# Robotics-Engineer-khy/ti5_isaacgym

Hardware: AMD Instinct MI355X
Metric: env-steps/sec at 8192 envs, t1_dh_stand, 1/2/4/8 MI355X; obs/reward parity (higher is better)
Workload: dtype f32

## Files before the change

ti5_isaacgym_amd/csrc/t1env_dyn6.hip:

```cpp
#include <hip/hip_runtime.h>

#define T1_CONTACT_ONE_COPY

#ifdef T1_PROBE_SIMD
__device__ unsigned g_t1_simd6[4096][8];
#endif
#ifdef T1_PROBE_CLOCK
__device__ unsigned long long g_t1_clock6[4];
constexpr int T1_WGSUM6_N = 4 + 6;
__device__ unsigned long long g_t1_wgtime6[4096][4];
__device__ unsigned long long g_t1_wgsum6[4096][T1_WGSUM6_N];
#define T1_CLOCK_WAIT_BEGIN() const unsigned long long t1c_w0 = __builtin_amdgcn_s_memtime();
#define T1_CLOCK_SHIFT_END(wi)                                                     \
  if ((threadIdx.x & 63) == 0 && blockIdx.x < 4096 && (wi) >= 0)                   \
    atomicAdd(&g_t1_wgsum6[blockIdx.x][4 + (wi)], __builtin_amdgcn_s_memtime() - t1c_w0);
#define T1_CLOCK_LOOP_END()                                                        \
  if (threadIdx.x == 0 && blockIdx.x < 4096) g_t1_wgtime6[blockIdx.x][3] = __builtin_amdgcn_s_memrealtime();
#define T1_CLOCK_WAIT_END(k)                                                       \
  if (threadIdx.x == 0 && blockIdx.x < 4096)                                       \
    atomicAdd(&g_t1_wgsum6[blockIdx.x][k], __builtin_amdgcn_s_memtime() - t1c_w0);
#define T1_CLOCK_BEGIN()                                                           \
  unsigned long long t1c_cyc0 = 0, t1c_rt0 = 0;                                    \
  if (threadIdx.x == 0) {                                                          \
    t1c_cyc0 = __builtin_amdgcn_s_memtime();                                       \
    t1c_rt0 = __builtin_amdgcn_s_memrealtime();                                    \
    if (blockIdx.x < 4096) { g_t1_wgtime6[blockIdx.x][0] = t1c_rt0; g_t1_wgtime6[blockIdx.x][2] = 0; } \
  }
#define T1_CLOCK_END()                                                             \
  if (threadIdx.x == 0) {                                                          \
    const unsigned long long c1 = __builtin_amdgcn_s_memtime(), r1 = __builtin_amdgcn_s_memrealtime(); \
    atomicAdd(&g_t1_clock6[0], c1 - t1c_cyc0);                                     \
    atomicAdd(&g_t1_clock6[1], r1 - t1c_rt0);                                      \
    atomicAdd(&g_t1_clock6[2], 1ull);                                              \
    if (blockIdx.x < 4096) {                                                       \
      g_t1_wgtime6[blockIdx.x][1] = r1;                                            \
      atomicAdd(&g_t1_wgsum6[blockIdx.x][0], c1 - t1c_cyc0);                       \
    }                                                                              \
  }                                                                                \
  T1_CLOCK_WAVE_END();
#define T1_CLOCK_WAVE_END()                                                        \
  if ((threadIdx.x & 63) == 0 && blockIdx.x < 4096)                                \
    atomicMax(&g_t1_wgtime6[blockIdx.x][2], (unsigned long long)__builtin_amdgcn_s_memrealtime());
constexpr int T1_TAIL6_N = 16;
__device__ unsigned long long g_t1_tail6[4096][T1_TAIL6_N];
#define T1_CLOCK_STAMP(k)                                                          \
  if ((threadIdx.x & 63) == 0 && blockIdx.x < 4096)                                \
    g_t1_tail6[blockIdx.x][k] = __builtin_amdgcn_s_memrealtime();
#else
#define T1_CLOCK_BEGIN() ((void)0)
#define T1_CLOCK_END() ((void)0)
#define T1_CLOCK_WAVE_END() ((void)0)
#define T1_CLOCK_WAIT_BEGIN() ((void)0)
#define T1_CLOCK_WAIT_END(k) ((void)0)
#define T1_CLOCK_SHIFT_END(wi) ((void)0)
#define T1_CLOCK_LOOP_END() ((void)0)
#define T1_CLOCK_STAMP(k) ((void)0)
#endif

#define T1_PROF_WAVES 8
#define T1_PROF_NAME(x) x##6
#include "t1env_prof.h"

#include "t1_dyn5.h"
#include "t1env_device.h"
#include "t1env_internal.h"
#include "t1env_postphys.h"
// ... 14 lines not shown
constexpr int SHIFT6_WAVES = __builtin_popcount(SHIFT6_MASK);
static_assert((SHIFT6_MASK & 0x11) == 0, "W0 / W4 (the core chain's SIMD) do not shift");

struct Dyn6Lds {
  DynModel model;
  Rows4<Q_N> st;
  Rows4<WB_N> wb;
  SubspaceRows sj;
  Rows4<R_N> w1;
  Rows4<XCH> wc[WC_N];
  PdStage<64> pd;
  float cap[CAP5_N][64];
  float act[12][NE6];
  float epi[EPI_N][NE6];
  float fr[FR_N][NE6];
  float vish[64];
  float vift[64];
  float amx[4][64];
  LegParams<float> pl[64];
  BaseParams<float> pb[64];
  float rtf[2][3][64];
  float rsf[2][3][64];
  uint32_t e2;
};
T1_ROWS_ALIGNED(Dyn6Lds, st);
T1_ROWS_ALIGNED(Dyn6Lds, wb);
T1_ROWS_ALIGNED(Dyn6Lds, sj);
T1_ROWS_ALIGNED(Dyn6Lds, w1);
T1_ROWS_ALIGNED(Dyn6Lds, wc);
static_assert(sizeof(Rows4<XCH>) % 16 == 0 && alignof(Dyn6Lds) % 16 == 0, "every wc[i], and the struct itself");

template <int F, int H, bool HALF>
__device__ __forceinline__ void shift_chunk_elems(const uint8_t* in0, uint8_t* out0, uint32_t i, uint32_t nel) {
  constexpr uint32_t ROW = F * H, PER = HALF ? 8 : 4;
#pragma unroll 1
  for (uint32_t k = 0; k < PER; ++k) {
    const uint32_t e = i + k;
    if (e < nel && e % ROW < ROW - F) {
      if constexpr (HALF)
        reinterpret_cast<uint16_t*>(out0)[e] = reinterpret_cast<const uint16_t*>(in0)[e + F];
      else
        reinterpret_cast<float*>(out0)[e] = reinterpret_cast<const float*>(in0)[e + F];
    }
  }
}
template <int F, int H, bool HALF>
__device__ __forceinline__ void shp_range(int64_t total, int64_t r0, int64_t r1, int sl, int nsl, uint32_t& lo,
// ... 492 lines not shown
    halves(vi_b, vl, vr);
    __syncthreads();
    V3<float> fb = v3<float>(0.0f, 0.0f, 0.0f);
    {
      BaseState<float> sb;
      float q[NLEG], qd[NLEG];
      read_state_rows(lds.st, lane, sb, q, qd);
      if (leg == 0) {
      BaseFrame<float> F;
      base_frame(sb, F);
      const float vt0 = restitution_target(M, eg, vl), vt1 = restitution_target(M, eg, vr);
      fb = body_contact_force(M, T, 0, F.R0, v3<float>(0, 0, 0), F.abs, F.V0, mu, vt0 > vt1 ? vt0 : vt1);
      }
    }
    __syncthreads();
    if (leg == 0) {
      if (active) {
        float* cf = B.contact_forces + (size_t)n * 39;
        cf[0] = fb.x; cf[1] = fb.y; cf[2] = fb.z;
      }
      if constexpr (FUSED) { lds.fr[F_CFB][e] = fb.x; lds.fr[F_CFB + 1][e] = fb.y; lds.fr[F_CFB + 2][e] = fb.z; }
    }
    T1_PROF_MARK(10);
    if constexpr (FUSED) __syncthreads();
    T1_CLOCK_WAVE_END();
    T1_PROF_END();
    return;
  }

  if (role != 0) {
    T1_PROF_MARK(21);
    const int wi = shift6_index(role);
    const float mu = 0.5f * (B.friction[n] + M.ground_friction);
    const float mu_self = B.friction[n];
    const float eg = ground_restitution(M, B.restitution[n]);
    if (FUSED && wave >= 4) stage_epilogue_inputs<NE6, 256>(B, N, (int)r0, (int)threadIdx.x - 256, lds.epi);
    T1_PROF_MARK(22);
    const int bsh = 1 + 6 * leg + K_SHANK, bft = 1 + 6 * leg + K_FOOT;
    const int half = role >= 4 ? 1 : 0;
    if (role == 1) {
      LegParams<float> PL;
      load_leg_params(M, B, n, j0, PL);
      ShiftHold hold;
      ShiftWalk walk;
      shp_begin(S, r0, r1, nsub, wi, lane, walk, hold);
      for (int sub = 0; sub < nsub; ++sub) {
        T1_PROF_MARK(4);
// ... 164 lines not shown
            const float w[3] = {lds.cap[2 * NLEG + 4][lane], lds.cap[2 * NLEG + 5][lane], lds.cap[2 * NLEG + 6][lane]};
            capture_imu(quat, w, imu_dst);
          }
        }
      }
      __syncthreads();
      T1_PROF_MARK(11);
      if (role == 6) {
        float* cf = B.contact_forces + (size_t)n * 39;
#pragma unroll
        for (int s = 0; s < 2; ++s) {
          const int b = s == 0 ? bsh : bft;
          const float f[3] = {lds.rtf[s][0][lane] + lds.rsf[s][0][lane], lds.rtf[s][1][lane] + lds.rsf[s][1][lane],
                              lds.rtf[s][2][lane] + lds.rsf[s][2][lane]};
          if (active) { cf[b * 3 + 0] = f[0]; cf[b * 3 + 1] = f[1]; cf[b * 3 + 2] = f[2]; }
          if (FUSED && s == 1) {
            const int r = leg == 0 ? F_C0 : F_C1;
            lds.fr[r][e] = f[0]; lds.fr[r + 1][e] = f[1]; lds.fr[r + 2][e] = f[2];
          }
        }
      }
    }
    if constexpr (FUSED) {
      if (role == 1 && lane == 0) lds.e2 = 0u;
      __syncthreads();
      T1_PROF_MARK(12);
      if (role == 1)
        fused_epilogue_staged<POST_A_STATE, NE6, true, false>(M, C, B, A, S, FA, dyn_blocks, lane, lds.epi,
                                                                             lds.fr, lds.act, lds.act + NLEG, &lds.e2);
      else if (role == 2)
        fused_epilogue_obs<POST_OBS_PRIV, NE6>(M, C, B, A, lane, lds.epi, lds.fr, lds.act, lds.act + NLEG);
      else if (role == 3)
        fused_epilogue_obs<POST_OBS_ACTOR, NE6>(M, C, B, A, lane, lds.epi, lds.fr, lds.act, lds.act + NLEG);
      else if (wave >= 5)
        epilogue_zero_reset_rows<NE6>(C, B, S, lane, (int)threadIdx.x - 320, 192, lds.epi, lds.fr);
      T1_PROF_MARK(15);
    }
    T1_CLOCK_WAVE_END();
    T1_PROF_END();
    return;
  }

  BaseParams<float>& PB = lds.pb[lane];
  LegParams<float>& PL = lds.pl[lane];
  {
    BaseState<float> sb;
    float q[NLEG], qd[NLEG];
    BaseParams<float> pb;
    LegParams<float> pl;
    load_base_params(M, B, n, pb);
    load_leg_params(M, B, n, j0, pl);
    load_base_state(M, pb, B.root_states + (size_t)n * 13, sb);
    PB = pb;
    PL = pl;
#pragma unroll
    for (int k = 0; k < NLEG; ++k) {
      q[k] = B.dof_state[n * 24 + 2 * (j0 + k)];
      qd[k] = B.dof_state[n * 24 + 2 * (j0 + k) + 1];
// ... 120 lines not shown
  }
  float (*FR)[NE6] = FUSED ? lds.fr : nullptr;
  if constexpr (FUSED) {
#pragma unroll
    for (int k = 0; k < NLEG; ++k) {
      lds.fr[F_DOF + 2 * (j0 + k)][e] = q[k];
      lds.fr[F_DOF + 2 * (j0 + k) + 1][e] = qd[k];
    }
  }
  T1_PROF_MARK(8);
  __syncthreads();
  T1_PROF_MARK(9);
  {
    BaseFrame<float> F;
    base_frame(sb, F);
    leg_report_rigid<NE6>(M, B, PB, sb, F, q, qd, no, leg, active, e, FR);
  }
  T1_PROF_MARK(10);
  __syncthreads();
  T1_PROF_MARK(11);
  if constexpr (FUSED) {
    __syncthreads();
    T1_PROF_MARK(12);
    fused_epilogue_staged<POST_A_REWARDS, NE6, true, false>(M, C, B, A, S, FA, dyn_blocks, lane, lds.epi,
                                                                           lds.fr, lds.act, lds.act + NLEG, &lds.e2);
  }
  T1_CLOCK_END();
  T1_PROF_END();
}

#ifdef T1_PROBE_SIMD
extern "C" int t1env_debug_simd6(unsigned* out, int blocks) {
  return (int)hipMemcpyFromSymbol(out, HIP_SYMBOL(g_t1_simd6), sizeof(unsigned) * 8 * (size_t)blocks);
}
#endif

#ifdef T1_PROBE_CLOCK
extern "C" int t1env_debug_wgtime6(unsigned long long* out, int blocks) {
  return (int)hipMemcpyFromSymbol(out, HIP_SYMBOL(g_t1_wgtime6), sizeof(unsigned long long) * 4 * (size_t)blocks);
}
extern "C" int t1env_debug_tail6(unsigned long long* out, int blocks) {
  return (int)hipMemcpyFromSymbol(out, HIP_SYMBOL(g_t1_tail6), sizeof(unsigned long long) * T1_TAIL6_N * (size_t)blocks);
}
extern "C" int t1env_debug_wgsum6(unsigned long long* out, int blocks, int reset) {
  hipError_t e = hipMemcpyFromSymbol(out, HIP_SYMBOL(g_t1_wgsum6), sizeof(unsigned long long) * T1_WGSUM6_N * (size_t)blocks);
  if (e == hipSuccess && reset) {
    static unsigned long long zero[4096][T1_WGSUM6_N] = {};
    e = hipMemcpyToSymbol(HIP_SYMBOL(g_t1_wgsum6), zero, sizeof(zero));
// ... 29 lines not shown
```

ti5_isaacgym_amd/csrc/t1env_fused.h:

```cpp
#pragma once
#include "t1env_device.h"
#include "t1env_internal.h"
#include "t1env_postphys.h"

#ifndef T1_CLOCK_STAMP
#define T1_CLOCK_STAMP(k) ((void)0)
#endif

namespace t1 {

constexpr int SHIFT_UNIT = 8;
constexpr int K_SHANK = 3, K_FOOT = 5;
static_assert(T1_LEG_CONTACT_MASK == ((1 << K_SHANK) | (1 << K_FOOT)), "the step kernels assume shank + foot contacts");
constexpr int XCH = 27;

constexpr uint32_t HANDOFF_SHIFT = 1u, HANDOFF_DYN = 2u;
__device__ __forceinline__ uint32_t unit_handoff(uint32_t* word, uint32_t epoch, uint32_t bits) {
  const uint32_t tag = (epoch & 0x3fffffu) << 10;
  uint32_t old = __hip_atomic_load(word, __ATOMIC_RELAXED, __HIP_MEMORY_SCOPE_AGENT);
  for (;;) {
    const uint32_t nw = ((old & ~0x3ffu) == tag ? old : tag) | bits;
    if (__hip_atomic_compare_exchange_strong(word, &old, nw, __ATOMIC_RELAXED, __ATOMIC_RELAXED,
                                             __HIP_MEMORY_SCOPE_AGENT))
      return nw;
// ... 242 lines not shown
  while (todo) {
    const int l = __ffsll(todo) - 1;
    todo &= todo - 1;
    const int64_t row = (int64_t)blockIdx.x * NE + l;
    zero_history_row(S, row, t, nt);
    zero_span_wide(B.act_hist + row * 48, 48, t, nt);
    zero_span_wide(B.dof_hist + row * 96, 96, t, nt);
    zero_span_wide(B.imu_hist + row * 16, 16, t, nt);
  }
}

__device__ __forceinline__ void epilogue_reset_rest(const DynModel& M, const t1env_config& C, const t1env_buffers& B,
                                                    const t1env_step_args& A, int n, uint32_t genv, uint32_t ctr,
                                                    RngKey K, const float (&cmd)[4], float org[3], bool org_known,
                                                    bool zero_lag_rings) {
  reset_env_rest(M, C, B, n, K, org, org_known, false, true, zero_lag_rings);
  ObsIn O;
#pragma unroll
  for (int i = 0; i < 4; ++i) O.cmd[i] = cmd[i];
  reset_obs_inputs(M, C, K, O, false);
  if (resample_commands_r(C, A, O.el, O.gt, O.cmd, genv, ctr)) strow(B.commands + n * 4, O.cmd);
}

template <int PART, int NE, bool INWG, bool RESET_ROWS = true>
__device__ __forceinline__ void fused_epilogue_staged(const DynModel& M, const t1env_config& C, const t1env_buffers& B,
                                                      const t1env_step_args& A, const ShiftArgs& S,
                                                      const FusedArgs& FA, int dyn_blocks, int lane,
                                                      const float (*E)[NE], const float (*FR)[NE],
                                                      const float (*ACT0)[NE], const float (*ACT1)[NE],
                                                      uint32_t* e2_flag = nullptr) {
  const int N = C.num_envs;
  constexpr int TS = PART == POST_A_REWARDS ? 0 : 8;
  T1_CLOCK_STAMP(TS);
  const int e = lane % NE;
  const int n0 = lane < NE ? (int)blockIdx.x * NE + lane : N;
  const bool active = n0 < N;
  const int n = active ? n0 : N - 1;
  PostAIn X;
#pragma unroll
  for (int i = 0; i < 13; ++i) X.root[i] = FR[F_ROOT + i][e];
#pragma unroll
  for (int i = 0; i < 24; ++i) X.dof[i] = FR[F_DOF + i][e];
#pragma unroll
  for (int i = 0; i < 13; ++i) { X.f0[i] = FR[F_F0 + i][e]; X.f1[i] = FR[F_F1 + i][e]; }
#pragma unroll
  for (int i = 0; i < 2; ++i) { X.k0[i] = FR[F_K0 + i][e]; X.k1[i] = FR[F_K1 + i][e]; }
#pragma unroll
  for (int i = 0; i < 3; ++i) { X.cfb[i] = FR[F_CFB + i][e]; X.c0[i] = FR[F_C0 + i][e]; X.c1[i] = FR[F_C1 + i][e]; }
#pragma unroll
  for (int i = 0; i < 12; ++i) X.tq[i] = FR[F_TQ + i][e];
#pragma unroll
  for (int k = 0; k < NLEG; ++k) { X.a[k] = ACT0[k][e]; X.a[NLEG + k] = ACT1[k][e]; }
#pragma unroll
  for (int i = 0; i < 12; ++i) {
    X.la[i] = E[E_LA + i][e]; X.lla[i] = E[E_LLA + i][e];
    X.ldv[i] = E[E_LDV + i][e]; X.ref[i] = E[E_REF + i][e];
// ... 3 lines not shown
#pragma unroll
  for (int i = 0; i < 4; ++i) X.cmd[i] = E[E_CMD + i][e];
#pragma unroll
  for (int i = 0; i < 2; ++i) {
    X.at[i] = E[E_AT + i][e]; X.fh[i] = E[E_FH + i][e]; X.lfz[i] = E[E_LFZ + i][e];
    X.lc[i] = (uint8_t)__float_as_int(E[E_LC + i][e]);
  }
#pragma unroll
  for (int i = 0; i < 3; ++i) {
    X.ef[i] = E[E_EF + i][e]; X.et[i] = E[E_ET + i][e];
    X.gt[i] = __float_as_int(E[E_GT + i][e]);
  }
#pragma unroll
  for (int k = 0; k < T1_NREW; ++k) X.esum[k] = E[E_ESUM + k][e];
  X.el = (int64_t)(((uint64_t)(uint32_t)__float_as_int(E[E_EL + 1][e]) << 32) |
                   (uint32_t)__float_as_int(E[E_EL][e]));
  X.pl = (int64_t)(((uint64_t)(uint32_t)__float_as_int(E[E_PL + 1][e]) << 32) |
                   (uint32_t)__float_as_int(E[E_PL][e]));
  X.gstart = E[E_GS][e];
  BaseQ bq;
  float* const ep_row = FA.ep_part + (size_t)blockIdx.x * EP_PART_ROW;
  const bool in_level_sum = PART == POST_A_STATE && C.custom_origins && active;
  int level = in_level_sum ? B.terrain_levels[n] : 0;
  const bool do_reset = post_a_core<PART>(M, C, B, A, n0, X, bq, PART == POST_A_REWARDS ? ep_row : nullptr);
  T1_PROF_MARK(13);
  T1_CLOCK_STAMP(TS + 1);
  if constexpr (PART == POST_A_REWARDS) {
    if constexpr (RESET_ROWS) epilogue_handoff<NE, INWG>(C, S, FA, lane, do_reset, active);
    T1_CLOCK_STAMP(TS + 2);
    __builtin_amdgcn_s_waitcnt(0);
    T1_CLOCK_STAMP(TS + 3);
    if (e2_flag) {
      while (__hip_atomic_load(e2_flag, __ATOMIC_ACQUIRE, __HIP_MEMORY_SCOPE_WORKGROUP) == 0u) __builtin_amdgcn_s_sleep(1);
    } else {
      __syncthreads();
    }
    T1_CLOCK_STAMP(TS + 4);
    epilogue_finalize_parts(C, B, A, FA, dyn_blocks, lane);
    T1_CLOCK_STAMP(TS + 5);
    T1_PROF_MARK(15);
    return;
  }
  const uint32_t genv = (uint32_t)(C.env_offset + n);
  const uint32_t ctr = A.counter + 1u;
  const RngKey K = rng_key(C.seed, genv, ctr);
  float org[3];
  bool org_known = false;
  if (active && do_reset) {
    const float pos_cmd[4] = {X.root[0], X.root[1], X.cmd[0], X.cmd[1]};
    org_known = reset_curriculum(C, B, n, K, true, pos_cmd, org, level, in_level_sum);
  }
  if (!e2_flag && active && do_reset)
    epilogue_reset_rest(M, C, B, A, n, genv, ctr, K, X.cmd, org, org_known, RESET_ROWS);
  T1_PROF_MARK(14);
  T1_CLOCK_STAMP(TS + 2);
  wave_sum_store(ep_row + T1_ACC_LEVEL, in_level_sum ? (float)level : 0.0f);
  __builtin_amdgcn_s_waitcnt(0);
  T1_CLOCK_STAMP(TS + 3);
  if (e2_flag) {
    if (lane == 0) __hip_atomic_store(e2_flag, 1u, __ATOMIC_RELEASE, __HIP_MEMORY_SCOPE_WORKGROUP);
  } else {
    __syncthreads();
  }
  T1_CLOCK_STAMP(TS + 4);
  if (e2_flag && active && do_reset)
    epilogue_reset_rest(M, C, B, A, n, genv, ctr, K, X.cmd, org, org_known, RESET_ROWS);
  T1_CLOCK_STAMP(TS + 5);
  T1_PROF_MARK(15);
}

template <int PART, int NE>
__device__ __forceinline__ void fused_epilogue_obs(const DynModel& M, const t1env_config& C, const t1env_buffers& B,
                                                   const t1env_step_args& A, int lane, const float (*E)[NE],
                                                   const float (*FR)[NE], const float (*ACT0)[NE],
                                                   const float (*ACT1)[NE]) {
  static_assert(PART == POST_OBS_PRIV || PART == POST_OBS_ACTOR, "an observation part");
  constexpr bool PRIV = PART == POST_OBS_PRIV;
  const int e = lane % NE;
  const int n = (int)blockIdx.x * NE + lane;
  if (lane >= NE || n >= C.num_envs) return;
  const uint32_t genv = (uint32_t)(C.env_offset + n);
  const uint32_t ctr = A.counter + 1u;
  const RngKey K = rng_key(C.seed, genv, ctr);
  float ld[24], lraw[8];
  if constexpr (!PRIV)
    load_lagged(B, A, n, __float_as_int(E[E_DL][e]), __float_as_int(E[E_IL][e]), ld, lraw);
  ObsIn O;
#pragma unroll
  for (int i = 0; i < 4; ++i) O.cmd[i] = E[E_CMD + i][e];
// ... 149 lines not shown
```

ti5_isaacgym_amd/csrc/t1env_postphys.h:

```cpp
#pragma once
#include "t1env_device.h"

namespace t1 {

struct Phase {
  float sin_pos;
  float stance[2];
};

template <int K, typename T>
__device__ __forceinline__ void ldrow(T (&d)[K], const T* s) {
#pragma unroll
  for (int i = 0; i < K; ++i) d[i] = s[i];
}
template <int K, typename T>
__device__ __forceinline__ void strow(T* d, const T (&s)[K]) {
#pragma unroll
  for (int i = 0; i < K; ++i) d[i] = s[i];
}

__device__ __forceinline__ float phase_value(const t1env_config& C, int64_t phase_len, float gait_start, bool stand) {
  const float dtf = (float)(C.sim_dt * C.decimation);
  float ph = ((float)phase_len * dtf) / C.cycle_time;
  ph = ph - floorf(ph);
// ... 181 lines not shown
  }
  af[0] = af[1] = af[2] = 0.0f;
  ext_store = true;
  if (A.ext_force_call) {
    if (A.ext_force_first) {
      ef[0] = rand_float(-C.ext_force_max[0] / 2, C.ext_force_max[0], K, SLOT_EXT_FORCE + 0);
      ef[1] = rand_float(-C.ext_force_max[1], C.ext_force_max[1], K, SLOT_EXT_FORCE + 1);
      ef[2] = rand_float(-C.ext_force_max[2], C.ext_force_max[2], K, SLOT_EXT_FORCE + 2);
#pragma unroll
      for (int k = 0; k < 3; ++k)
        et[k] = rand_float(-C.ext_torque_max, C.ext_torque_max, K, SLOT_EXT_TORQUE + k);
    } else {
      const float st = is_stand(C, cmd) ? 1.0f : 0.0f;
      af[0] = ef[0] * st; af[1] = ef[1] * st; af[2] = ef[2] * st;
      ext_store = false;
    }
  } else {
    ef[0] = ef[1] = ef[2] = 0.0f;
    et[0] = et[1] = et[2] = 0.0f;
  }
  return cmd_dirty;
}

enum : int { POST_A_ALL = 0, POST_A_REWARDS = 1, POST_A_STATE = 2, POST_OBS_PRIV = 3, POST_OBS_ACTOR = 4 };
template <int PART = POST_A_ALL>
__device__ __forceinline__ bool post_a_core(const DynModel& M, const t1env_config& C, const t1env_buffers& B,
                                            const t1env_step_args& A, int n0, PostAIn& X, BaseQ& bq,
                                            float* ep_row = nullptr) {
  const bool live = n0 < C.num_envs;
  const int n = live ? n0 : C.num_envs - 1;
  const uint32_t genv = (uint32_t)(C.env_offset + n);
  const uint32_t ctr = A.counter + 1u;
  const RngKey K = rng_key(C.seed, genv, ctr);
  const size_t N = (size_t)C.num_envs;
  float (&root)[13] = X.root;
  const float (&dof)[24] = X.dof;
  const float (&f0)[13] = X.f0;
  const float (&f1)[13] = X.f1;
  const float (&k0)[2] = X.k0;
  const float (&k1)[2] = X.k1;
  const float (&cfb)[3] = X.cfb;
  const float (&c0)[3] = X.c0;
  const float (&c1)[3] = X.c1;
  const float (&a)[12] = X.a;
  const float (&la)[12] = X.la;
  const float (&lla)[12] = X.lla;
  const float (&lrv)[6] = X.lrv;
  const float (&ldv)[12] = X.ldv;
  const float (&tq)[12] = X.tq;
  const float (&ref)[12] = X.ref;
  float (&cmd)[4] = X.cmd;
  float (&esum)[T1_NREW] = X.esum;
  float (&at)[2] = X.at;
  float (&fh)[2] = X.fh;
  float (&lfz)[2] = X.lfz;
  float (&ef)[3] = X.ef;
  float (&et)[3] = X.et;
  uint8_t (&lc)[2] = X.lc;
  const int32_t (&gt)[3] = X.gt;
  const int64_t el = X.el + 1;
  int64_t pl = X.pl + 1;
  const float gstart = X.gstart;
  base_quantities_r(root, bq);
  const float* blv = bq.lin;
  const float* bav = bq.ang;
  const float* pg = bq.grav;
  const float* be = bq.euler;
  float fe[6];
  if constexpr (PART != POST_A_STATE) {
    const float q0[4] = {f0[3], f0[4], f0[5], f0[6]}, q1[4] = {f1[3], f1[4], f1[5], f1[6]};
    euler_xyz(q0, fe);
    euler_xyz(q1, fe + 3);
  }
  T1_PROF_MARK(16);
  float af[3];
  bool ext_store;
  const bool cmd_dirty = post_callback(C, A, genv, ctr, K, el, gt, cmd, root, ef, et, af, ext_store);
  T1_PROF_MARK(17);
  const bool term = norm3(cfb[0], cfb[1], cfb[2]) > 1.0f;
  const bool tout = (float)el > C.max_episode_length;
  const bool do_reset = live && (term || tout);
  const bool stand = is_stand(C, cmd);
  if (stand) pl = 0;
  const Phase ph = gait_phase(phase_value(C, pl, gstart, stand));
  const float dtf = (float)(C.sim_dt * C.decimation);
  const bool contact0 = c0[2] > 5.0f, contact1 = c1[2] > 5.0f;
  float r[T1_NREW];
  if constexpr (PART != POST_A_STATE) {
    {
      float t1s = 0.0f, t2s = 0.0f, t3s = 0.0f;
#pragma unroll
      for (int j = 0; j < 12; ++j) {
        const float d1 = (la[j] - a[j]) * 1.0f;
        const float d2 = ((a[j] + lla[j]) - 2.0f * la[j]) * 1.0f;
        t1s += d1 * d1;
        t2s += d2 * d2;
        t3s += fabsf(a[j] * 1.0f);
      }
      r[T1_REW_ACTION_SMOOTHNESS] = (t1s + t2s) + 0.05f * t3s;
    }
    {
      float s = 0.0f;
#pragma unroll
      for (int i = 0; i < 6; ++i) { const float d = lrv[i] - root[7 + i]; s += d * d; }
      r[T1_REW_BASE_ACC] = expf(-sqrtf(s) * 3.0f);
    }
    {
      const float mh = (f0[2] * ph.stance[0] + f1[2] * ph.stance[1]) / (ph.stance[0] + ph.stance[1]);
      const float bh = root[2] - (mh - 0.05f);
      r[T1_REW_BASE_HEIGHT] = expf(-fabsf(bh - C.base_height_target) * 100.0f);
    }
    r[T1_REW_COLLISION] = norm3(cfb[0], cfb[1], cfb[2]) > 0.1f ? 1.0f : 0.0f;
    {
      float jd[12], s = 0.0f;
#pragma unroll
      for (int j = 0; j < 12; ++j) { jd[j] = dof[2 * j] - M.default_dof_pos[j]; s += jd[j] * jd[j]; }
      float yr = norm3(jd[0], jd[1], jd[5]) + norm3(jd[6], jd[7], jd[11]);
      yr = clampf(yr - 0.1f, 0.0f, 50.0f);
      r[T1_REW_DEFAULT_JOINT_POS] = expf(-yr * 100.0f) - 0.01f * sqrtf(s);
    }
    {
      float s5 = 0.0f, s6 = 0.0f;
#pragma unroll
      for (int j = 0; j < 12; ++j) {
        const float d = (ldv[j] - dof[2 * j + 1]) / dtf;
        s5 += d * d;
        s6 += dof[2 * j + 1] * dof[2 * j + 1];
      }
      r[T1_REW_DOF_ACC] = s5;
      r[T1_REW_DOF_VEL] = s6;
    }
    r[T1_REW_DOF_VEL_LIMITS] = 0.0f;
    if (C.reward_scales[T1_REW_DOF_VEL_LIMITS] != 0.0f) {
      float s = 0.0f;
#pragma unroll
      for (int j = 0; j < 12; ++j) {
        const float lim = (j == 4 || j == 9) ? 10.0f : M.vel_limit[j];
        s += clampf(fabsf(dof[2 * j + 1]) - lim * C.soft_dof_vel_limit, 0.0f, 1.0f);
      }
      r[T1_REW_DOF_VEL_LIMITS] = s;
    }
    r[T1_REW_FEET_AIR_TIME] = 0.0f;
    if (C.reward_scales[T1_REW_FEET_AIR_TIME] != 0.0f) {
      float sm0 = ph.stance[0], sm1 = ph.stance[1];
      if (norm3(cmd[0], cmd[1], cmd[2]) < 0.05f) { sm0 = 1.0f; sm1 = 1.0f; }
      const bool filt0 = contact0 || sm0 > 0.0f || lc[0];
      const bool filt1 = contact1 || sm1 > 0.0f || lc[1];
      lc[0] = contact0; lc[1] = contact1;
      const bool first0 = at[0] > 0.0f && filt0, first1 = at[1] > 0.0f && filt1;
      const float a0 = at[0] + dtf, a1 = at[1] + dtf;
      const float air0 = clampf(a0, 0.0f, 0.5f) * (first0 ? 1.0f : 0.0f);
      const float air1 = clampf(a1, 0.0f, 0.5f) * (first1 ? 1.0f : 0.0f);
      at[0] = a0 * (filt0 ? 0.0f : 1.0f);
      at[1] = a1 * (filt1 ? 0.0f : 1.0f);
      r[T1_REW_FEET_AIR_TIME] = air0 + air1;
    }
    r[T1_REW_FEET_CLEARANCE] = 0.0f;
    if (C.reward_scales[T1_REW_FEET_CLEARANCE] != 0.0f) {
      const float z0 = f0[2], z1 = f1[2];
      const float h0 = fh[0] + (z0 - lfz[0]), h1 = fh[1] + (z1 - lfz[1]);
      lfz[0] = z0; lfz[1] = z1;
      const float sw0 = 1.0f - ph.stance[0], sw1 = 1.0f - ph.stance[1];
      const float rp0 = (h0 > C.target_feet_height && h0 < C.target_feet_height_max) ? 1.0f : 0.0f;
      const float rp1 = (h1 > C.target_feet_height && h1 < C.target_feet_height_max) ? 1.0f : 0.0f;
      r[T1_REW_FEET_CLEARANCE] = rp0 * sw0 + rp1 * sw1;
      fh[0] = h0 * (contact0 ? 0.0f : 1.0f);
      fh[1] = h1 * (contact1 ? 0.0f : 1.0f);
    }
    r[T1_REW_FEET_CONTACT_FORCES] = clampf(norm3(c0[0], c0[1], c0[2]) - C.max_contact_force, 0.0f, 400.0f) +
           clampf(norm3(c1[0], c1[1], c1[2]) - C.max_contact_force, 0.0f, 400.0f);
    {
      float sm0 = ph.stance[0], sm1 = ph.stance[1];
      if (stand) { sm0 = 1.0f; sm1 = 1.0f; }
      const float q0 = ((contact0 ? 1.0f : 0.0f) == sm0) ? 1.0f : -0.3f;
      const float q1 = ((contact1 ? 1.0f : 0.0f) == sm1) ? 1.0f : -0.3f;
      r[T1_REW_FEET_CONTACT_NUMBER] = (q0 + q1) / 2.0f;
    }
    {
      const float fd = norm2(f0[0] - f1[0], f0[1] - f1[1]);
      const float kd = norm2(k0[0] - k1[0], k0[1] - k1[1]);
      const float fmn = clampf(fd - C.foot_min_dist, -0.5f, 0.0f), fmx = clampf(fd - C.foot_max_dist, 0.0f, 0.5f);
      const float kmn = clampf(kd - C.knee_min_dist, -0.5f, 0.0f), kmx = clampf(kd - C.knee_max_dist, 0.0f, 0.5f);
      r[T1_REW_FEET_DISTANCE] = (expf(-fabsf(fmn) * 100.0f) + expf(-fabsf(fmx) * 100.0f)) / 2.0f;
      r[T1_REW_KNEE_DISTANCE] = (expf(-fabsf(kmn) * 100.0f) + expf(-fabsf(kmx) * 100.0f)) / 2.0f;
    }
    {
      const float rot = fe[1] * fe[1] + fe[4] * fe[4];
      const float x = rot / 1.0f;
      r[T1_REW_FEET_ROTATION] = 1.0f * expf(-(x * x));
    }
    r[T1_REW_FEET_STUMBLE] = 0.0f;
    if (C.reward_scales[T1_REW_FEET_STUMBLE] != 0.0f) {
      const bool st0 = norm2(c0[0], c0[1]) > 5.0f * fabsf(c0[2]), st1 = norm2(c1[0], c1[1]) > 5.0f * fabsf(c1[2]);
      r[T1_REW_FEET_STUMBLE] = (st0 || st1) ? 1.0f : 0.0f;
    }
    {
      const float s0 = sqrtf(norm2(f0[10], f0[11])), s1 = sqrtf(norm2(f1[10], f1[11]));
      r[T1_REW_FOOT_SLIP] = s0 * (contact0 ? 1.0f : 0.0f) + s1 * (contact1 ? 1.0f : 0.0f);
    }
    {
      float s = 0.0f;
#pragma unroll
      for (int j = 0; j < 12; ++j) {
        const float tgt = stand ? M.default_dof_pos[j] : ref[j];
        const float d = dof[2 * j] - tgt;
        s += d * d;
      }
      const float nr = sqrtf(s);
      r[T1_REW_JOINT_POS] = stand ? 1.0f : expf(-2.0f * nr) - 0.2f * clampf(nr, 0.0f, 0.5f);
    }
    {
      const float sp = fabsf(blv[0]), cm = fabsf(cmd[0]);
      const bool low = sp < 0.5f * cm, high = sp > 1.2f * cm, ok = !(low || high);
      const bool mis = signf(blv[0]) != signf(cmd[0]);
      float v = 0.0f;
      if (low) v = -1.0f;
      if (high) v = 0.0f;
      if (ok) v = 1.2f;
      if (mis) v = -2.0f;
      r[T1_REW_LOW_SPEED] = v * (fabsf(cmd[0]) > 0.05f ? 1.0f : 0.0f);
    }
    {
      const float qm = expf(-(fabsf(be[0]) + fabsf(be[1])) * 10.0f);
      const float o = expf(-norm2(pg[0], pg[1]) * 20.0f);
      r[T1_REW_ORIENTATION] = (qm + o) / 2.0f;
    }
    {
      const int idx[8] = {0, 1, 2, 3, 5, 6, 7, 8};
      const float w[10] = {2.0f, 2.0f, 1.0f, 1.0f, 1.0f, 2.0f, 2.0f, 1.0f, 1.0f, 1.0f};
      float s = 0.0f;
#pragma unroll
      for (int k = 0; k < 8; ++k) {
        const float e = (dof[2 * idx[k]] - M.default_dof_pos[idx[k]]) * w[k];
        s += e * e;
      }
      const float e8 = fe[1] * w[8], e9 = fe[4] * w[9];
      s += e8 * e8;
      s += e9 * e9;
      r[T1_REW_STAND_STILL] = stand ? expf(-s) : 0.0f;
    }
    r[T1_REW_STAND_SYSMETRY] = 0.0f;
    if (C.reward_scales[T1_REW_STAND_SYSMETRY] != 0.0f) {
      float s = 0.0f;
#pragma unroll
      for (int k = 0; k < 4; ++k) { const float d = dof[2 * k] - dof[2 * (5 + k)]; s += d * d; }
      r[T1_REW_STAND_SYSMETRY] = stand ? expf(-s) : 0.0f;
    }
    r[T1_REW_TERMINATION] = 0.0f;
    {
      float s = 0.0f;
#pragma unroll
      for (int j = 0; j < 12; ++j) s += tq[j] * tq[j];
      r[T1_REW_TORQUES] = s;
    }
    {
      const float le = norm2(cmd[0] - blv[0], cmd[1] - blv[1]);
      const float ae = fabsf(cmd[2] - bav[2]);
      r[T1_REW_TRACK_VEL_HARD] = (expf(-le * 10.0f) + expf(-ae * 10.0f)) / 2.0f - 0.2f * (le + ae);
    }
    {
      const float d = cmd[2] - bav[2];
      r[T1_REW_TRACKING_ANG_VEL] = stand ? expf(-fabsf(d) * (C.tracking_sigma * 2.0f)) : expf(-(d * d) * C.tracking_sigma);
    }
    {
      const float dx = cmd[0] - blv[0], dy = cmd[1] - blv[1];
      r[T1_REW_TRACKING_LIN_VEL] = stand ? expf(-(fabsf(dx) + fabsf(dy)) * (C.tracking_sigma * 2.0f))
                    : expf(-(dx * dx + dy * dy) * C.tracking_sigma);
    }
    {
      const float lm = expf(-(blv[2] * blv[2]) * 10.0f);
      const float am = expf(-norm2(bav[0], bav[1]) * 5.0f);
      r[T1_REW_VEL_MISMATCH_EXP] = (lm + am) / 2.0f;
    }
  }
  T1_PROF_MARK(18);
  float rew = 0.0f, contrib[T1_NREW];
  if constexpr (PART != POST_A_STATE) {
#pragma unroll
    for (int k = 0; k < T1_NREW; ++k) {
      if (k == T1_REW_TERMINATION) continue;
      const float v = r[k] * C.reward_scales[k];
      rew = rew + v;
      esum[k] = esum[k] + v;
    }
    if (C.only_positive_rewards) rew = fmaxf(rew, 0.0f);
    if (C.reward_scales[T1_REW_TERMINATION] != 0.0f) {
      const float v = ((do_reset && !tout) ? 1.0f : 0.0f) * C.reward_scales[T1_REW_TERMINATION];
      rew = rew + v;
      esum[T1_REW_TERMINATION] = esum[T1_REW_TERMINATION] + v;
    }
#pragma unroll
    for (int k = 0; k < T1_NREW; ++k) contrib[k] = do_reset ? esum[k] : 0.0f;
  }
  T1_PROF_MARK(19);
  if (live) {
    if constexpr (PART != POST_A_REWARDS) {
      B.episode_length_buf[n] = el;
      B.phase_length_buf[n] = pl;
// ... 433 lines not shown
```

Measured before the change: 72.68 million.

## Split reward-term evaluation across idle helper waves and widen per-env reset writes

Reward terms that keep no state are spread over four otherwise idle waves (4-7). Each helper writes its terms into a new LDS array and signals completion through a workgroup-scope atomic counter, which the main reward wave spins on before summing. The reset tail now walks the resetting lanes through a ballot loop and uses all 64 lanes to write each env's rows, replacing the one-lane-per-env loop. This shortens the serial epilogue on the critical wave, at the cost of more LDS, a spin-wait, and helper waves redoing the shared input loads.

Result: faster. 73.70 million (median of 6 runs) (+1.4%).

```diff
diff --git a/ti5_isaacgym_amd/csrc/t1env_dyn6.hip b/ti5_isaacgym_amd/csrc/t1env_dyn6.hip
--- a/ti5_isaacgym_amd/csrc/t1env_dyn6.hip
+++ b/ti5_isaacgym_amd/csrc/t1env_dyn6.hip
@@ -41,7 +41,7 @@
 #define T1_CLOCK_WAVE_END()                                                        \
   if ((threadIdx.x & 63) == 0 && blockIdx.x < 4096)                                \
     atomicMax(&g_t1_wgtime6[blockIdx.x][2], (unsigned long long)__builtin_amdgcn_s_memrealtime());
-constexpr int T1_TAIL6_N = 16;
+constexpr int T1_TAIL6_N = 20;
 __device__ unsigned long long g_t1_tail6[4096][T1_TAIL6_N];
 #define T1_CLOCK_STAMP(k)                                                          \
   if ((threadIdx.x & 63) == 0 && blockIdx.x < 4096)                                \
@@ -102,7 +102,22 @@
   float rtf[2][3][64];
   float rsf[2][3][64];
   uint32_t e2;
+  uint32_t rwn;
+  float rw[T1_NREW][NE6];
 };
+constexpr uint32_t REW6_W4 = (1u << T1_REW_LOW_SPEED) | (1u << T1_REW_ORIENTATION) | (1u << T1_REW_TRACK_VEL_HARD) |
+                             (1u << T1_REW_TRACKING_ANG_VEL) | (1u << T1_REW_TRACKING_LIN_VEL) |
+                             (1u << T1_REW_VEL_MISMATCH_EXP);
+constexpr uint32_t REW6_W5 = (1u << T1_REW_BASE_ACC) | (1u << T1_REW_DEFAULT_JOINT_POS) | (1u << T1_REW_JOINT_POS) |
+                             (1u << T1_REW_DOF_VEL_LIMITS) | (1u << T1_REW_STAND_SYSMETRY);
+constexpr uint32_t REW6_W6 = (1u << T1_REW_ACTION_SMOOTHNESS) | (1u << T1_REW_DOF_ACC) | (1u << T1_REW_DOF_VEL) |
+                             (1u << T1_REW_TORQUES);
+constexpr uint32_t REW6_W7 = (1u << T1_REW_FEET_DISTANCE) | (1u << T1_REW_KNEE_DISTANCE) | (1u << T1_REW_FOOT_SLIP) |
+                             (1u << T1_REW_FEET_CONTACT_FORCES);
+constexpr uint32_t REW6_HELPED = REW6_W4 | REW6_W5 | REW6_W6 | REW6_W7;
+constexpr uint32_t REW6_HELPERS = 4;
+static_assert(__builtin_popcount(REW6_HELPED) == __builtin_popcount(REW6_W4) + __builtin_popcount(REW6_W5) +
+              __builtin_popcount(REW6_W6) + __builtin_popcount(REW6_W7), "a term has one owner");
 T1_ROWS_ALIGNED(Dyn6Lds, st);
 T1_ROWS_ALIGNED(Dyn6Lds, wb);
 T1_ROWS_ALIGNED(Dyn6Lds, sj);
@@ -641,7 +656,11 @@
       if constexpr (FUSED) { lds.fr[F_CFB][e] = fb.x; lds.fr[F_CFB + 1][e] = fb.y; lds.fr[F_CFB + 2][e] = fb.z; }
     }
     T1_PROF_MARK(10);
-    if constexpr (FUSED) __syncthreads();
+    if constexpr (FUSED) {
+      __syncthreads();
+      fused_epilogue_staged<POST_A_REW_HELPER, NE6, true, false, REW6_W4>(
+          M, C, B, A, S, FA, dyn_blocks, lane, lds.epi, lds.fr, lds.act, lds.act + NLEG, nullptr, lds.rw, &lds.rwn);
+    }
     T1_CLOCK_WAVE_END();
     T1_PROF_END();
     return;
@@ -852,7 +871,7 @@
       }
     }
     if constexpr (FUSED) {
-      if (role == 1 && lane == 0) lds.e2 = 0u;
+      if (role == 1 && lane == 0) { lds.e2 = 0u; lds.rwn = 0u; }
       __syncthreads();
       T1_PROF_MARK(12);
       if (role == 1)
@@ -862,8 +881,18 @@
         fused_epilogue_obs<POST_OBS_PRIV, NE6>(M, C, B, A, lane, lds.epi, lds.fr, lds.act, lds.act + NLEG);
       else if (role == 3)
         fused_epilogue_obs<POST_OBS_ACTOR, NE6>(M, C, B, A, lane, lds.epi, lds.fr, lds.act, lds.act + NLEG);
-      else if (wave >= 5)
+      else if (wave >= 5) {
+        if (role == 5)
+          fused_epilogue_staged<POST_A_REW_HELPER, NE6, true, false, REW6_W5>(
+              M, C, B, A, S, FA, dyn_blocks, lane, lds.epi, lds.fr, lds.act, lds.act + NLEG, nullptr, lds.rw, &lds.rwn);
+        else if (role == 6)
+          fused_epilogue_staged<POST_A_REW_HELPER, NE6, true, false, REW6_W6>(
+              M, C, B, A, S, FA, dyn_blocks, lane, lds.epi, lds.fr, lds.act, lds.act + NLEG, nullptr, lds.rw, &lds.rwn);
+        else
+          fused_epilogue_staged<POST_A_REW_HELPER, NE6, true, false, REW6_W7>(
+              M, C, B, A, S, FA, dyn_blocks, lane, lds.epi, lds.fr, lds.act, lds.act + NLEG, nullptr, lds.rw, &lds.rwn);
         epilogue_zero_reset_rows<NE6>(C, B, S, lane, (int)threadIdx.x - 320, 192, lds.epi, lds.fr);
+      }
       T1_PROF_MARK(15);
     }
     T1_CLOCK_WAVE_END();
@@ -1030,8 +1059,9 @@
   if constexpr (FUSED) {
     __syncthreads();
     T1_PROF_MARK(12);
-    fused_epilogue_staged<POST_A_REWARDS, NE6, true, false>(M, C, B, A, S, FA, dyn_blocks, lane, lds.epi,
-                                                                           lds.fr, lds.act, lds.act + NLEG, &lds.e2);
+    fused_epilogue_staged<POST_A_REWARDS, NE6, true, false, REW_ALL & ~REW6_HELPED>(
+        M, C, B, A, S, FA, dyn_blocks, lane, lds.epi, lds.fr, lds.act, lds.act + NLEG, &lds.e2, lds.rw, &lds.rwn,
+        REW6_HELPERS);
   }
   T1_CLOCK_END();
   T1_PROF_END();
diff --git a/ti5_isaacgym_amd/csrc/t1env_fused.h b/ti5_isaacgym_amd/csrc/t1env_fused.h
--- a/ti5_isaacgym_amd/csrc/t1env_fused.h
+++ b/ti5_isaacgym_amd/csrc/t1env_fused.h
@@ -288,16 +288,87 @@
   if (resample_commands_r(C, A, O.el, O.gt, O.cmd, genv, ctr)) strow(B.commands + n * 4, O.cmd);
 }
 
-template <int PART, int NE, bool INWG, bool RESET_ROWS = true>
+template <int K, typename T>
+__device__ __forceinline__ T row_sel(const T (&v)[K], int i) {
+  T r = T(0);
+#pragma unroll
+  for (int k = 0; k < K; ++k) r = i == k ? v[k] : r;
+  return r;
+}
+
+__device__ __forceinline__ void epilogue_reset_rest_wide(const DynModel& M, const t1env_config& C,
+                                                         const t1env_buffers& B, const t1env_step_args& A, int n,
+                                                         uint32_t genv, uint32_t ctr, RngKey K, const float (&cmd)[4],
+                                                         const float (&org)[3], int lane) {
+  ObsIn R;
+#pragma unroll
+  for (int i = 0; i < 4; ++i) R.cmd[i] = cmd[i];
+  reset_obs_inputs(M, C, K, R, false);
+  const bool cmd_dirty = resample_commands_r(C, A, R.el, R.gt, R.cmd, genv, ctr);
+  if (lane < NVIMP) B.contact_vimp[(size_t)n * NVIMP + lane] = 0.0f;
+  if (lane < 24) {
+    const int j = lane >> 1;
+    const float q = M.default_dof_pos[j] + rand_float(-C.reset_dof_range, C.reset_dof_range, K, SLOT_RESET_DOF + j);
+    B.dof_state[n * 24 + lane] = (lane & 1) ? 0.0f : q;
+  }
+  if (lane < 13) {
+    float r = M.base_init_state[lane];
+    if (lane < 3) r += row_sel(org, lane);
+    if (C.custom_origins && lane < 2) {
+      const float p3 = C.reset_xy_range;
+      r += rand_float(-p3, p3, K, SLOT_RESET_ROOT_XY + lane);
+    }
+    B.root_states[n * 13 + lane] = r;
+  }
+#pragma unroll
+  for (int p = 0; p < 2; ++p) {
+    const int i = lane + 64 * p;
+    if (i < 72) {
+      const int a = i / 12, j = i - 12 * a;
+      const float lo = a == 0 ? C.motor_offset_range[0] : a == 1 ? C.kp_mult_range[0] : a == 2 ? C.kd_mult_range[0]
+                     : a == 3 ? C.coulomb_range[0] : a == 4 ? C.viscous_range[0] : C.armature_range[j][0];
+      const float hi = a == 0 ? C.motor_offset_range[1] : a == 1 ? C.kp_mult_range[1] : a == 2 ? C.kd_mult_range[1]
+                     : a == 3 ? C.coulomb_range[1] : a == 4 ? C.viscous_range[1] : C.armature_range[j][1];
+      const uint32_t slot = a == 0 ? SLOT_DR_OFFSET : a == 1 ? SLOT_DR_KP : a == 2 ? SLOT_DR_KD
+                          : a == 3 ? SLOT_DR_COULOMB : a == 4 ? SLOT_DR_VISCOUS : SLOT_DR_ARMATURE;
+      const float u = rand_float(lo, hi, K, slot + (a == 5 && C.armature_shared ? 0 : j));
+      const float v = a == 1 ? u * M.p_gains[j] : a == 2 ? u * M.d_gains[j] : u;
+      float* const dst = a == 0 ? B.motor_offsets : a == 1 ? B.kp : a == 2 ? B.kd
+                       : a == 3 ? B.coulomb : a == 4 ? B.viscous : B.armature;
+      dst[n * 12 + j] = v;
+    }
+  }
+  if (lane < 12) B.actions[n * 12 + lane] = 0.0f;
+  if (lane < 3) {
+    B.gait_time[n * 3 + lane] = row_sel(R.gt, lane);
+    B.base_lin_vel[n * 3 + lane] = row_sel(R.bq.lin, lane);
+    B.base_ang_vel[n * 3 + lane] = row_sel(R.bq.ang, lane);
+    B.projected_gravity[n * 3 + lane] = row_sel(R.bq.grav, lane);
+    B.base_euler_xyz[n * 3 + lane] = row_sel(R.bq.euler, lane);
+  }
+  if (lane == 0) {
+    if (cmd_dirty) strow(B.commands + n * 4, R.cmd);
+    B.lag_timestep[n] = rand_int(C.lag_range[0], C.lag_range[1] + 1, K, SLOT_LAG_ACTION);
+    B.dof_lag_timestep[n] = R.dl;
+    B.imu_lag_timestep[n] = R.il;
+    B.episode_length_buf[n] = 0;
+    B.phase_length_buf[n] = 0;
+    B.reset_buf[n] = 1;
+    B.gait_start[n] = R.gstart;
+  }
+}
+
+template <int PART, int NE, bool INWG, bool RESET_ROWS = true, uint32_t TERMS = REW_ALL>
 __device__ __forceinline__ void fused_epilogue_staged(const DynModel& M, const t1env_config& C, const t1env_buffers& B,
                                                       const t1env_step_args& A, const ShiftArgs& S,
                                                       const FusedArgs& FA, int dyn_blocks, int lane,
                                                       const float (*E)[NE], const float (*FR)[NE],
                                                       const float (*ACT0)[NE], const float (*ACT1)[NE],
-                                                      uint32_t* e2_flag = nullptr) {
+                                                      uint32_t* e2_flag = nullptr, float (*RW)[NE] = nullptr,
+                                                      uint32_t* rw_count = nullptr, uint32_t rw_helpers = 0) {
   const int N = C.num_envs;
   constexpr int TS = PART == POST_A_REWARDS ? 0 : 8;
-  T1_CLOCK_STAMP(TS);
+  if constexpr (PART != POST_A_REW_HELPER) T1_CLOCK_STAMP(TS);
   const int e = lane % NE;
   const int n0 = lane < NE ? (int)blockIdx.x * NE + lane : N;
   const bool active = n0 < N;
@@ -347,7 +418,13 @@
   float* const ep_row = FA.ep_part + (size_t)blockIdx.x * EP_PART_ROW;
   const bool in_level_sum = PART == POST_A_STATE && C.custom_origins && active;
   int level = in_level_sum ? B.terrain_levels[n] : 0;
-  const bool do_reset = post_a_core<PART>(M, C, B, A, n0, X, bq, PART == POST_A_REWARDS ? ep_row : nullptr);
+  RewDeal D;
+  if (RW) {
+    D.rows = &RW[0][0]; D.stride = NE; D.col = e; D.owner = lane < NE;
+    D.count = rw_count; D.helpers = rw_helpers;
+  }
+  const bool do_reset = post_a_core<PART, TERMS>(M, C, B, A, n0, X, bq, PART == POST_A_REWARDS ? ep_row : nullptr, D);
+  if constexpr (PART == POST_A_REW_HELPER) return;
   T1_PROF_MARK(13);
   T1_CLOCK_STAMP(TS + 1);
   if constexpr (PART == POST_A_REWARDS) {
@@ -388,8 +465,24 @@
     __syncthreads();
   }
   T1_CLOCK_STAMP(TS + 4);
-  if (e2_flag && active && do_reset)
-    epilogue_reset_rest(M, C, B, A, n, genv, ctr, K, X.cmd, org, org_known, RESET_ROWS);
+  if (e2_flag) {
+    if (active && do_reset && !org_known)
+#pragma unroll
+      for (int i = 0; i < 3; ++i) org[i] = B.env_origins[n * 3 + i];
+    unsigned long long todo = __ballot(active && do_reset);
+    while (todo) {
+      const int l = __ffsll(todo) - 1;
+      todo &= todo - 1;
+      const int nl = (int)blockIdx.x * NE + l;
+      const RngKey Kl = {(uint32_t)__builtin_amdgcn_readlane((int)K.h, l)};
+      float cmd_l[4], org_l[3];
+#pragma unroll
+      for (int i = 0; i < 4; ++i) cmd_l[i] = __int_as_float(__builtin_amdgcn_readlane(__float_as_int(X.cmd[i]), l));
+#pragma unroll
+      for (int i = 0; i < 3; ++i) org_l[i] = __int_as_float(__builtin_amdgcn_readlane(__float_as_int(org[i]), l));
+      epilogue_reset_rest_wide(M, C, B, A, nl, (uint32_t)(C.env_offset + nl), ctr, Kl, cmd_l, org_l, lane);
+    }
+  }
   T1_CLOCK_STAMP(TS + 5);
   T1_PROF_MARK(15);
 }
diff --git a/ti5_isaacgym_amd/csrc/t1env_postphys.h b/ti5_isaacgym_amd/csrc/t1env_postphys.h
--- a/ti5_isaacgym_amd/csrc/t1env_postphys.h
+++ b/ti5_isaacgym_amd/csrc/t1env_postphys.h
@@ -1,5 +1,9 @@
 #pragma once
 #include "t1env_device.h"
+
+#ifndef T1_CLOCK_STAMP
+#define T1_CLOCK_STAMP(k) ((void)0)
+#endif
 
 namespace t1 {
 
@@ -227,11 +231,28 @@
   return cmd_dirty;
 }
 
-enum : int { POST_A_ALL = 0, POST_A_REWARDS = 1, POST_A_STATE = 2, POST_OBS_PRIV = 3, POST_OBS_ACTOR = 4 };
-template <int PART = POST_A_ALL>
+enum : int { POST_A_ALL = 0, POST_A_REWARDS = 1, POST_A_STATE = 2, POST_OBS_PRIV = 3, POST_OBS_ACTOR = 4,
+             POST_A_REW_HELPER = 5 };
+constexpr uint32_t REW_ALL = (1u << T1_NREW) - 1u;
+constexpr uint32_t REW_HELPER_TERMS =
+    REW_ALL & ~((1u << T1_REW_FEET_AIR_TIME) | (1u << T1_REW_FEET_CLEARANCE) | (1u << T1_REW_FEET_ROTATION) |
+                (1u << T1_REW_STAND_STILL) | (1u << T1_REW_TERMINATION));
+constexpr bool rew_in(uint32_t terms, int k) { return ((terms >> k) & 1u) != 0u; }
+struct RewDeal {
+  float* rows = nullptr;
+  int stride = 0, col = 0;
+  bool owner = false;
+  uint32_t* count = nullptr;
+  uint32_t helpers = 0;
+};
+template <int PART = POST_A_ALL, uint32_t TERMS = REW_ALL>
 __device__ __forceinline__ bool post_a_core(const DynModel& M, const t1env_config& C, const t1env_buffers& B,
                                             const t1env_step_args& A, int n0, PostAIn& X, BaseQ& bq,
-                                            float* ep_row = nullptr) {
+                                            float* ep_row = nullptr, const RewDeal D = RewDeal{}) {
+  static_assert(rew_in(TERMS, T1_REW_DOF_ACC) == rew_in(TERMS, T1_REW_DOF_VEL) &&
+                rew_in(TERMS, T1_REW_FEET_DISTANCE) == rew_in(TERMS, T1_REW_KNEE_DISTANCE), "evaluated in one block");
+  static_assert(PART == POST_A_REWARDS || PART == POST_A_REW_HELPER || TERMS == REW_ALL, "only the fused reward pass is dealt");
+  static_assert(PART != POST_A_REW_HELPER || (TERMS & ~REW_HELPER_TERMS) == 0u, "a helper's terms keep no state");
   const bool live = n0 < C.num_envs;
   const int n = live ? n0 : C.num_envs - 1;
   const uint32_t genv = (uint32_t)(C.env_offset + n);
@@ -272,7 +293,7 @@
   const float* pg = bq.grav;
   const float* be = bq.euler;
   float fe[6];
-  if constexpr (PART != POST_A_STATE) {
+  if constexpr (PART != POST_A_STATE && PART != POST_A_REW_HELPER) {
     const float q0[4] = {f0[3], f0[4], f0[5], f0[6]}, q1[4] = {f1[3], f1[4], f1[5], f1[6]};
     euler_xyz(q0, fe);
     euler_xyz(q1, fe + 3);
@@ -292,7 +313,7 @@
   const bool contact0 = c0[2] > 5.0f, contact1 = c1[2] > 5.0f;
   float r[T1_NREW];
   if constexpr (PART != POST_A_STATE) {
-    {
+    if constexpr (rew_in(TERMS, T1_REW_ACTION_SMOOTHNESS)) {
       float t1s = 0.0f, t2s = 0.0f, t3s = 0.0f;
 #pragma unroll
       for (int j = 0; j < 12; ++j) {
@@ -304,19 +325,19 @@
       }
       r[T1_REW_ACTION_SMOOTHNESS] = (t1s + t2s) + 0.05f * t3s;
     }
-    {
+    if constexpr (rew_in(TERMS, T1_REW_BASE_ACC)) {
       float s = 0.0f;
 #pragma unroll
       for (int i = 0; i < 6; ++i) { const float d = lrv[i] - root[7 + i]; s += d * d; }
       r[T1_REW_BASE_ACC] = expf(-sqrtf(s) * 3.0f);
     }
-    {
+    if constexpr (rew_in(TERMS, T1_REW_BASE_HEIGHT)) {
       const float mh = (f0[2] * ph.stance[0] + f1[2] * ph.stance[1]) / (ph.stance[0] + ph.stance[1]);
       const float bh = root[2] - (mh - 0.05f);
       r[T1_REW_BASE_HEIGHT] = expf(-fabsf(bh - C.base_height_target) * 100.0f);
     }
-    r[T1_REW_COLLISION] = norm3(cfb[0], cfb[1], cfb[2]) > 0.1f ? 1.0f : 0.0f;
-    {
+    if constexpr (rew_in(TERMS, T1_REW_COLLISION)) r[T1_REW_COLLISION] = norm3(cfb[0], cfb[1], cfb[2]) > 0.1f ? 1.0f : 0.0f;
+    if constexpr (rew_in(TERMS, T1_REW_DEFAULT_JOINT_POS)) {
       float jd[12], s = 0.0f;
 #pragma unroll
       for (int j = 0; j < 12; ++j) { jd[j] = dof[2 * j] - M.default_dof_pos[j]; s += jd[j] * jd[j]; }
@@ -324,7 +345,7 @@
       yr = clampf(yr - 0.1f, 0.0f, 50.0f);
       r[T1_REW_DEFAULT_JOINT_POS] = expf(-yr * 100.0f) - 0.01f * sqrtf(s);
     }
-    {
+    if constexpr (rew_in(TERMS, T1_REW_DOF_ACC)) {
       float s5 = 0.0f, s6 = 0.0f;
 #pragma unroll
       for (int j = 0; j < 12; ++j) {
@@ -336,7 +357,7 @@
       r[T1_REW_DOF_VEL] = s6;
     }
     r[T1_REW_DOF_VEL_LIMITS] = 0.0f;
-    if (C.reward_scales[T1_REW_DOF_VEL_LIMITS] != 0.0f) {
+    if (rew_in(TERMS, T1_REW_DOF_VEL_LIMITS) && C.reward_scales[T1_REW_DOF_VEL_LIMITS] != 0.0f) {
       float s = 0.0f;
 #pragma unroll
       for (int j = 0; j < 12; ++j) {
@@ -346,7 +367,7 @@
       r[T1_REW_DOF_VEL_LIMITS] = s;
     }
     r[T1_REW_FEET_AIR_TIME] = 0.0f;
-    if (C.reward_scales[T1_REW_FEET_AIR_TIME] != 0.0f) {
+    if (rew_in(TERMS, T1_REW_FEET_AIR_TIME) && C.reward_scales[T1_REW_FEET_AIR_TIME] != 0.0f) {
       float sm0 = ph.stance[0], sm1 = ph.stance[1];
       if (norm3(cmd[0], cmd[1], cmd[2]) < 0.05f) { sm0 = 1.0f; sm1 = 1.0f; }
       const bool filt0 = contact0 || sm0 > 0.0f || lc[0];
@@ -361,7 +382,7 @@
       r[T1_REW_FEET_AIR_TIME] = air0 + air1;
     }
     r[T1_REW_FEET_CLEARANCE] = 0.0f;
-    if (C.reward_scales[T1_REW_FEET_CLEARANCE] != 0.0f) {
+    if (rew_in(TERMS, T1_REW_FEET_CLEARANCE) && C.reward_scales[T1_REW_FEET_CLEARANCE] != 0.0f) {
       const float z0 = f0[2], z1 = f1[2];
       const float h0 = fh[0] + (z0 - lfz[0]), h1 = fh[1] + (z1 - lfz[1]);
       lfz[0] = z0; lfz[1] = z1;
@@ -372,16 +393,16 @@
       fh[0] = h0 * (contact0 ? 0.0f : 1.0f);
       fh[1] = h1 * (contact1 ? 0.0f : 1.0f);
     }
-    r[T1_REW_FEET_CONTACT_FORCES] = clampf(norm3(c0[0], c0[1], c0[2]) - C.max_contact_force, 0.0f, 400.0f) +
+    if constexpr (rew_in(TERMS, T1_REW_FEET_CONTACT_FORCES)) r[T1_REW_FEET_CONTACT_FORCES] = clampf(norm3(c0[0], c0[1], c0[2]) - C.max_contact_force, 0.0f, 400.0f) +
            clampf(norm3(c1[0], c1[1], c1[2]) - C.max_contact_force, 0.0f, 400.0f);
-    {
+    if constexpr (rew_in(TERMS, T1_REW_FEET_CONTACT_NUMBER)) {
       float sm0 = ph.stance[0], sm1 = ph.stance[1];
       if (stand) { sm0 = 1.0f; sm1 = 1.0f; }
       const float q0 = ((contact0 ? 1.0f : 0.0f) == sm0) ? 1.0f : -0.3f;
       const float q1 = ((contact1 ? 1.0f : 0.0f) == sm1) ? 1.0f : -0.3f;
       r[T1_REW_FEET_CONTACT_NUMBER] = (q0 + q1) / 2.0f;
     }
-    {
+    if constexpr (rew_in(TERMS, T1_REW_FEET_DISTANCE)) {
       const float fd = norm2(f0[0] - f1[0], f0[1] - f1[1]);
       const float kd = norm2(k0[0] - k1[0], k0[1] - k1[1]);
       const float fmn = clampf(fd - C.foot_min_dist, -0.5f, 0.0f), fmx = clampf(fd - C.foot_max_dist, 0.0f, 0.5f);
@@ -389,21 +410,21 @@
       r[T1_REW_FEET_DISTANCE] = (expf(-fabsf(fmn) * 100.0f) + expf(-fabsf(fmx) * 100.0f)) / 2.0f;
       r[T1_REW_KNEE_DISTANCE] = (expf(-fabsf(kmn) * 100.0f) + expf(-fabsf(kmx) * 100.0f)) / 2.0f;
     }
-    {
+    if constexpr (rew_in(TERMS, T1_REW_FEET_ROTATION)) {
       const float rot = fe[1] * fe[1] + fe[4] * fe[4];
       const float x = rot / 1.0f;
       r[T1_REW_FEET_ROTATION] = 1.0f * expf(-(x * x));
     }
     r[T1_REW_FEET_STUMBLE] = 0.0f;
-    if (C.reward_scales[T1_REW_FEET_STUMBLE] != 0.0f) {
+    if (rew_in(TERMS, T1_REW_FEET_STUMBLE) && C.reward_scales[T1_REW_FEET_STUMBLE] != 0.0f) {
       const bool st0 = norm2(c0[0], c0[1]) > 5.0f * fabsf(c0[2]), st1 = norm2(c1[0], c1[1]) > 5.0f * fabsf(c1[2]);
       r[T1_REW_FEET_STUMBLE] = (st0 || st1) ? 1.0f : 0.0f;
     }
-    {
+    if constexpr (rew_in(TERMS, T1_REW_FOOT_SLIP)) {
       const float s0 = sqrtf(norm2(f0[10], f0[11])), s1 = sqrtf(norm2(f1[10], f1[11]));
       r[T1_REW_FOOT_SLIP] = s0 * (contact0 ? 1.0f : 0.0f) + s1 * (contact1 ? 1.0f : 0.0f);
     }
-    {
+    if constexpr (rew_in(TERMS, T1_REW_JOINT_POS)) {
       float s = 0.0f;
 #pragma unroll
       for (int j = 0; j < 12; ++j) {
@@ -414,7 +435,7 @@
       const float nr = sqrtf(s);
       r[T1_REW_JOINT_POS] = stand ? 1.0f : expf(-2.0f * nr) - 0.2f * clampf(nr, 0.0f, 0.5f);
     }
-    {
+    if constexpr (rew_in(TERMS, T1_REW_LOW_SPEED)) {
       const float sp = fabsf(blv[0]), cm = fabsf(cmd[0]);
       const bool low = sp < 0.5f * cm, high = sp > 1.2f * cm, ok = !(low || high);
       const bool mis = signf(blv[0]) != signf(cmd[0]);
@@ -425,12 +446,12 @@
       if (mis) v = -2.0f;
       r[T1_REW_LOW_SPEED] = v * (fabsf(cmd[0]) > 0.05f ? 1.0f : 0.0f);
     }
-    {
+    if constexpr (rew_in(TERMS, T1_REW_ORIENTATION)) {
       const float qm = expf(-(fabsf(be[0]) + fabsf(be[1])) * 10.0f);
       const float o = expf(-norm2(pg[0], pg[1]) * 20.0f);
       r[T1_REW_ORIENTATION] = (qm + o) / 2.0f;
     }
-    {
+    if constexpr (rew_in(TERMS, T1_REW_STAND_STILL)) {
       const int idx[8] = {0, 1, 2, 3, 5, 6, 7, 8};
       const float w[10] = {2.0f, 2.0f, 1.0f, 1.0f, 1.0f, 2.0f, 2.0f, 1.0f, 1.0f, 1.0f};
       float s = 0.0f;
@@ -445,40 +466,57 @@
       r[T1_REW_STAND_STILL] = stand ? expf(-s) : 0.0f;
     }
     r[T1_REW_STAND_SYSMETRY] = 0.0f;
-    if (C.reward_scales[T1_REW_STAND_SYSMETRY] != 0.0f) {
+    if (rew_in(TERMS, T1_REW_STAND_SYSMETRY) && C.reward_scales[T1_REW_STAND_SYSMETRY] != 0.0f) {
       float s = 0.0f;
 #pragma unroll
       for (int k = 0; k < 4; ++k) { const float d = dof[2 * k] - dof[2 * (5 + k)]; s += d * d; }
       r[T1_REW_STAND_SYSMETRY] = stand ? expf(-s) : 0.0f;
     }
     r[T1_REW_TERMINATION] = 0.0f;
-    {
+    if constexpr (rew_in(TERMS, T1_REW_TORQUES)) {
       float s = 0.0f;
 #pragma unroll
       for (int j = 0; j < 12; ++j) s += tq[j] * tq[j];
       r[T1_REW_TORQUES] = s;
     }
-    {
+    if constexpr (rew_in(TERMS, T1_REW_TRACK_VEL_HARD)) {
       const float le = norm2(cmd[0] - blv[0], cmd[1] - blv[1]);
       const float ae = fabsf(cmd[2] - bav[2]);
       r[T1_REW_TRACK_VEL_HARD] = (expf(-le * 10.0f) + expf(-ae * 10.0f)) / 2.0f - 0.2f * (le + ae);
     }
-    {
+    if constexpr (rew_in(TERMS, T1_REW_TRACKING_ANG_VEL)) {
       const float d = cmd[2] - bav[2];
       r[T1_REW_TRACKING_ANG_VEL] = stand ? expf(-fabsf(d) * (C.tracking_sigma * 2.0f)) : expf(-(d * d) * C.tracking_sigma);
     }
-    {
+    if constexpr (rew_in(TERMS, T1_REW_TRACKING_LIN_VEL)) {
       const float dx = cmd[0] - blv[0], dy = cmd[1] - blv[1];
       r[T1_REW_TRACKING_LIN_VEL] = stand ? expf(-(fabsf(dx) + fabsf(dy)) * (C.tracking_sigma * 2.0f))
                     : expf(-(dx * dx + dy * dy) * C.tracking_sigma);
     }
-    {
+    if constexpr (rew_in(TERMS, T1_REW_VEL_MISMATCH_EXP)) {
       const float lm = expf(-(blv[2] * blv[2]) * 10.0f);
       const float am = expf(-norm2(bav[0], bav[1]) * 5.0f);
       r[T1_REW_VEL_MISMATCH_EXP] = (lm + am) / 2.0f;
     }
   }
   T1_PROF_MARK(18);
+  if constexpr (PART == POST_A_REW_HELPER) {
+    if (D.owner)
+#pragma unroll
+      for (int k = 0; k < T1_NREW; ++k)
+        if (rew_in(TERMS, k)) D.rows[k * D.stride + D.col] = r[k];
+    if ((threadIdx.x & 63) == 0) __hip_atomic_fetch_add(D.count, 1u, __ATOMIC_RELEASE, __HIP_MEMORY_SCOPE_WORKGROUP);
+    T1_CLOCK_STAMP(10 + (int)(threadIdx.x >> 6));
+    return do_reset;
+  }
+  if constexpr (PART == POST_A_REWARDS && TERMS != REW_ALL) {
+    T1_CLOCK_STAMP(6);
+    while (__hip_atomic_load(D.count, __ATOMIC_ACQUIRE, __HIP_MEMORY_SCOPE_WORKGROUP) != D.helpers) __builtin_amdgcn_s_sleep(1);
+    T1_CLOCK_STAMP(7);
+#pragma unroll
+    for (int k = 0; k < T1_NREW; ++k)
+      if (!rew_in(TERMS, k) && k != T1_REW_TERMINATION) r[k] = D.rows[k * D.stride + D.col];
+  }
   float rew = 0.0f, contrib[T1_NREW];
   if constexpr (PART != POST_A_STATE) {
 #pragma unroll
```
